# tsolomko/SWCompression

Hardware: AMD Instinct MI355X
Metric: decompressed GiB/s (higher is better)
Workload: dtype u8; 1 GPU; 100000 x 64 KiB gzip members (BASELINE configs[1]; 4096 distinct, tiled at distinct addresses); codec=deflate, units_per_gpu=100000, unit_bytes=65536, compressed_bytes_per_gpu=2122936095, decompressed_bytes_per_gpu=6553600000, parallelism=1 x independent shards (weak scaling)

## Files before the change

### swcompression_amd/csrc/inflate_sync.h

```cpp
#ifndef SWC_INFLATE_SYNC_H
#define SWC_INFLATE_SYNC_H

#include "inflate_lane.h"
#include "simt.h"
#include "sync_round.h"

namespace swc {
namespace inflate {

#ifndef SWC_SYNC_LIT_BITS
#define SWC_SYNC_LIT_BITS 10
#endif
constexpr int kSyncLitBits = SWC_SYNC_LIT_BITS, kSyncDistBits = 8;
constexpr uint32_t kSyncChunk = SWC_SYNC_CHUNK;
constexpr uint32_t kSyncRound = 64u * kSyncChunk;
constexpr uint32_t kSyncStage = (kSyncRound + 32u + 15u) & ~15u;
constexpr uint32_t kPosFail = 0xFFFFFFFFu;
#ifndef SWC_SYNC_WALK_BACK
#define SWC_SYNC_WALK_BACK 128
#endif
#ifndef SWC_COPY_REC
#define SWC_COPY_REC 16
#define SWC_COPY_LIT 8
#endif
constexpr uint32_t kSyncWalkBack = SWC_SYNC_WALK_BACK;
static_assert(kSyncChunk % 4 == 0 && kSyncChunk >= 36, "sub-chunks are whole dwords");

#ifndef SWC_SYNC_NO_PAIRS
#define SWC_SYNC_NO_PAIRS 0
#endif
constexpr uint32_t kEntLenBit = (uint32_t)kSyncLitBits + 2u;
constexpr uint32_t kEntNotLen = ((1u << (kSyncLitBits - kSyncDistBits)) - 1u) << (kSyncDistBits + 2), kEntLen = 1u << kEntLenBit, kEntLit = 1u << 13, kEntDist = 1u << 29, kEntStop = 1u << 30, kEntTog = 1u << 31;
static_assert(kSyncLitBits > kSyncDistBits && kEntLenBit <= 12u, "the entry keeps bits 10 .. 12 for the table switch");
constexpr uint32_t kEntBaseShift = 14, kEntPosMask = kEntTog | kEntStop | 31u;
constexpr uint32_t kLitMask4 = ((1u << kSyncLitBits) - 1u) << 2, kDistMask4 = ((1u << kSyncDistBits) - 1u) << 2;
static_assert(kEntLen == 4u << kSyncLitBits, "the length flag is the byte offset of the distance table");
static_assert((kLitMask4 & ~kEntNotLen) == kDistMask4, "the masks differ in the not-length bits");
constexpr uint32_t kInvLit = 2u | kEntNotLen | kEntStop, kInvDist = kInvLit | kEntTog;
constexpr uint32_t kEntShShift = 23, kEntPairBit = 28, kEntPair = SWC_SYNC_NO_PAIRS ? 0u : 1u << kEntPairBit, kEntPairLenShift = 16, kPairLenMax = 127;
SWC_HD uint32_t make_entry(uint32_t clen, uint32_t ext, uint32_t kind, uint32_t mant, uint32_t sh) {
    const uint32_t c = (clen + ext + 2u) | ((clen + 2u) << 5);
    const uint32_t v = SWC_SYNC_NO_PAIRS ? (mant << sh) << kEntBaseShift : (mant << kEntBaseShift) | (sh << kEntShShift);
    return kind == 1 ? c | kEntNotLen | kEntLit | v
         : kind == 2 ? c | kEntLen | kEntTog | v
         : kind == 3 ? c | kEntNotLen | kEntStop
                     : c | kEntNotLen | kEntDist | kEntTog | v;
}
SWC_HD uint32_t ent_bits(uint32_t e) { return (e & 31u) - 2u; }
SWC_HD uint32_t ent_code_bits(uint32_t e) { return ((e >> 5) & 31u) - 2u; }
SWC_HD bool ent_is_eob(uint32_t e) { return (e & kEntStop) != 0u && (e & 31u) > 2u; }
SWC_HD bool ent_is_link(uint32_t e) { return (e & kEntPosMask) == 0u; }
SWC_HD bool ent_is_pair(uint32_t e) { return (e & kEntPair) != 0u; }
SWC_HD uint32_t ent_pair_len(uint32_t e) { return bfe32(e, kEntPairLenShift, 7); }
SWC_HD uint32_t ent_base(uint32_t e) {
    if (SWC_SYNC_NO_PAIRS) return bfe32(e, kEntBaseShift, 15);
    return bfe32(e, kEntBaseShift, ent_is_pair(e) ? 2u : 9u) << bfe32(e, kEntShShift, 4);
}
SWC_HD uint32_t pair_entry(uint32_t e, uint32_t idx, const uint32_t* dlut) {
    if (SWC_SYNC_NO_PAIRS || ent_is_link(e) || (e & (kEntLen | kEntStop)) != kEntLen) return 0u;
    const uint32_t nl = ent_bits(e), cl = ent_code_bits(e);
    if (nl >= (uint32_t)kSyncLitBits) return 0u;
    const uint32_t r = (uint32_t)kSyncLitBits - nl;
    const uint32_t len = ent_base(e) + ((idx >> cl) & ((1u << (nl - cl)) - 1u));
    if (len > kPairLenMax) return 0u;
    const uint32_t de = dlut[(idx >> nl) & ((1u << kSyncDistBits) - 1u)];
    if (ent_is_link(de) || (de & (kEntDist | kEntStop)) != kEntDist) return 0u;
    const uint32_t d = ent_code_bits(de);
    if (d > r) return 0u;
    const uint32_t c2 = nl + d + 2u, n2 = c2 + (ent_bits(de) - d);
    return n2 | (c2 << 5) | kEntNotLen | kEntDist | kEntPair | (len << kEntPairLenShift) | (de & ((3u << kEntBaseShift) | (15u << kEntShShift)));
}

SWC_HD uint32_t entry_of_symbol(bool dist, uint32_t sym, uint32_t d) {
    if (!dist) {
        if (sym < 256) return make_entry(d, 0, 1, sym, 0);
        if (sym == 256) return make_entry(d, 0, 3, 0, 0);
        if (sym > 285) return kInvLit;
        const uint32_t s = sym - 257u;
        const uint32_t e = s < 8 || s == 28 ? 0u : (s >> 2) - 1u;
        const uint32_t base = s < 8 ? 3u + s : s == 28 ? 258u : 3u + ((4u + (s & 3u)) << e);
        return make_entry(d, e, 2, base, 0);
    }
    if (sym > 29) return kInvDist;
    const uint32_t e = sym < 4 ? 0u : (sym >> 1) - 1u;
    return make_entry(d, e, 0, sym < 4 ? sym : 2u + (sym & 1u), e);
}

constexpr int kAuxLim = 0, kAuxSlot = 16, kAuxStart = 32, kAuxCount = 48 , kAuxOver = 49, kAuxTable = 52;
constexpr int kAuxLit = 0, kAuxDist = kAuxTable, kAuxWords = 2 * kAuxTable;
constexpr uint32_t kSpillSyms = 512, kSpillSub = 1536, kSubLds = 184, kSubMax = (uint32_t)(lzr::kProvSpillBytes - kSpillSub) / 4u;
constexpr uint32_t kSymDist = 288;
static_assert(kAuxWords * 4 <= (int)kSpillSyms && kSpillSyms + 2 * (288 + 32) <= kSpillSub && kSubMax < 4096u, "spill layout");

struct SyncLds {
    alignas(16) uint8_t stage[kSyncStage];
    uint32_t lut[(1 << kSyncLitBits) + (1 << kSyncDistBits)];
    uint32_t sub[kSubLds];
};
#if SWC_SYNC_CHUNK == 68 && SWC_SYNC_LIT_BITS == 10
static_assert(sizeof(SyncLds) == 10240, "16 waves per CU: the wave's LDS must stay within 160 KB / 16");
#endif
constexpr uint32_t kHdrLens = 0;
constexpr uint32_t kHdrRun = 320;
constexpr uint32_t kHdrClLut = 512;
constexpr uint32_t kHdrSorted = 640;
constexpr uint32_t kHdrRank = 1280;
constexpr uint32_t kHdrIn = 1280;
constexpr uint32_t kHdrPt = 1280;
constexpr uint32_t kHdrTab = 3840;
static_assert(kHdrTab + 2 * 33 * 4 <= kSyncStage && kHdrPt + 2 * 1280 <= kHdrTab, "header scratch fits the stage");

enum { kSyncEob = 0, kSyncBail = 1, kSyncBailCap = 2 };
#if defined(SWC_HOST_EMULATION)
inline uint64_t g_sync_stats[8];
#define SWC_SYNC_STAT(i, n) (g_sync_stats[i] += (n))
inline uint64_t g_sync_iters = 0, g_sync_wave[4] = {0, 0, 0, 0}, g_sync_passmax = 0, g_sync_it0 = 0;
inline uint8_t g_sync_long[4096];
#define SWC_SYNC_ITER() (g_sync_iters++)
#define SWC_SYNC_LONG() (g_sync_long[(g_sync_iters - 1 - g_sync_it0) & 4095] = 1)
#define SWC_SYNC_LANE_BEGIN(first) if (first) { g_sync_passmax = 0; for (auto& h_ : g_sync_long) h_ = 0; } g_sync_it0 = g_sync_iters;
#define SWC_SYNC_LANE_END(last, k) { if (g_sync_iters - g_sync_it0 > g_sync_passmax) g_sync_passmax = g_sync_iters - g_sync_it0; if (last) { g_sync_wave[k] += g_sync_passmax; for (auto h_ : g_sync_long) g_sync_wave[3] += h_; } }
#else
#define SWC_SYNC_STAT(i, n) ((void)0)
#define SWC_SYNC_ITER() ((void)0)
#define SWC_SYNC_LONG() ((void)0)
#define SWC_SYNC_LANE_BEGIN(first)
#define SWC_SYNC_LANE_END(last, k)
#endif
enum { kFlagEob = 1u, kFlagFail = 2u, kFlagTrap = 4u, kFlagSlow = 8u };
#if defined(SWC_PROFILE) && defined(__HIP_DEVICE_COMPILE__)
struct SyncProf {
    uint64_t acc[16] = {0, 0, 0, 0, 0, 0, 0, 0, 0, 0, 0, 0, 0, 0, 0, 0};
    uint64_t tlast = 0;
};
#define SWC_SP(pp, k) { const uint64_t t_ = __builtin_readcyclecounter(); (pp).acc[k] += t_ - (pp).tlast; (pp).tlast = t_; }
#define SWC_SPC(pp, k, n) ((pp).acc[k] += (n))
#else
struct SyncProf {};
#define SWC_SP(pp, k)
#define SWC_SPC(pp, k, n)
#endif

struct SubTab {
    const SWC_AS_GLOBAL uint32_t* g;
};
struct Spill {
    SWC_AS_GLOBAL uint32_t* aux;
    SWC_AS_GLOBAL uint16_t* syms;
    SWC_AS_GLOBAL uint32_t* sub;
};

SWC_D uint32_t stage_bits(const SyncLds* sl, uint32_t p) {
    const uint32_t* w = (const uint32_t*)(sl->stage + ((p >> 3) & 0x1FFCu));
    return funnel32(w[1], w[0], p);
}
SWC_D uint32_t long_lookup(const SyncLds* sl, const SubTab st, uint32_t bits4, uint32_t link) {
    const uint32_t idx = bfe32(bits4, link >> 10, link >> 5);
    const uint32_t at = (link >> 18) + idx;
    return st.g ? st.g[at] : sl->sub[at < kSubLds ? at : 0u];
}
SWC_D uint32_t entry_at(const SyncLds* sl, const SubTab st, uint32_t pos, bool dist, uint32_t& bits4) {
    bits4 = stage_bits(sl, pos);
    uint32_t e = *(const uint32_t*)((const uint8_t*)sl->lut + ((bits4 & (dist ? kDistMask4 : kLitMask4)) | (dist ? kEntLen : 0u)));
    if (ent_is_link(e)) e = long_lookup(sl, st, bits4, e);
    return e;
}

template <bool LIT>
SWC_D int decode_sym_canon(BitReader& br, const Spill sp) {
    const SWC_AS_GLOBAL uint32_t* tb = sp.aux + (LIT ? kAuxLit : kAuxDist);
    const uint32_t c15 = brev32(br.peek32()) >> 17;
    uint32_t len = 16, idx = 0;
    if (tb[kAuxOver] == 0) {
        len = 1;
#pragma unroll 1
        for (int d = 1; d <= 15; d++) len += c15 >= tb[kAuxLim + d] ? 1u : 0u;
        if (len > 15) return -1;
        idx = (tb[kAuxSlot + len] + (c15 >> (15 - len))) & 0xFFFFu;
    } else {
#pragma unroll 1
        for (uint32_t d = 1; d <= 15; d++) {
            const uint32_t st = tb[kAuxStart + d], cnt = (tb[kAuxStart + d + 1] - st) & 0xFFFFu;
            const uint32_t fst = d == 1 ? 0u : tb[kAuxLim + d - 1] >> (15 - d);
            const uint32_t k0 = ((c15 >> (15 - d)) - fst) & ((1u << d) - 1u);
            if (k0 < cnt) {
                len = d;
                idx = st + k0 + (((cnt - 1u - k0) >> d) << d);
                break;
            }
        }
        if (len > 15) return -1;
    }
    if (len > br.bc) return -1;
    br.consume(len);
    if (idx >= (LIT ? 288u : 32u)) return -1;
    return (int)sp.syms[(LIT ? 0u : kSymDist) + idx];
}

SWC_D int careful_step(Lane& ln, const Spill sp) {
    BitReader& br = ln.br;
    br.refill();
    const int sym = decode_sym_canon<true>(br, sp);
    if (sym < 0) return SWC_E_DEFLATE_SYMBOL_NOT_FOUND;
    if (sym < 256) {
        ln.put_byte((uint8_t)sym);
        return SWC_OK;
    }
    if (sym == 256) return -1;
    if (sym > 285) return SWC_E_DEFLATE_WRONG_SYMBOL;
    const uint32_t s = (uint32_t)sym - 257u;
    uint32_t length;
    if (s < 8) {
        length = 3 + s;
    } else if (s == 28) {
        length = 258;
    } else {
        const uint32_t e = (s >> 2) - 1;
        if (br.bc < e) return SWC_E_DEFLATE_SYMBOL_NOT_FOUND;
        length = 3 + ((4 + (s & 3)) << e) + br.bits(e);
    }
    br.refill();
    const int dc = decode_sym_canon<false>(br, sp);
    if (dc < 0) return SWC_E_DEFLATE_SYMBOL_NOT_FOUND;
    if (dc > 29) return SWC_E_DEFLATE_WRONG_SYMBOL;
    uint32_t distance;
    if (dc < 4) {
        distance = 1 + (uint32_t)dc;
    } else {
        const uint32_t e = ((uint32_t)dc >> 1) - 1;
        if (br.bc < e) return SWC_E_DEFLATE_SYMBOL_NOT_FOUND;
        distance = 1 + ((2 + ((uint32_t)dc & 1)) << e) + br.bits(e);
    }
    if ((uint64_t)distance > ln.pos) {
        const uint32_t over = distance - (uint32_t)ln.pos;
        if (over > ln.back) return SWC_E_REF_TRAP;
        if (over > ln.reach) ln.reach = over;
    }
    ln.emit_match(length, distance);
    return SWC_OK;
}

SWC_D void table_from_counts(const uint32_t* cnt, SWC_AS_GLOBAL uint32_t* tb, uint32_t* first, uint32_t* start) {
    uint32_t v = 0, off = 0, over = 0;
    tb[kAuxLim] = 0; tb[kAuxSlot] = 0; tb[kAuxStart] = 0;
    first[0] = 0; start[0] = 0;
#pragma unroll 1
    for (int d = 1; d <= 15; d++) {
        const uint32_t c = cnt[d];
        tb[kAuxLim + d] = (v + c) << (15 - d);
        if (c != 0 && v + c > (1u << d)) over = 1;
        tb[kAuxSlot + d] = (off - v) & 0xFFFFu;
        tb[kAuxStart + d] = off;
        first[d] = v;
        start[d] = off;
        off += c;
        v = (v + c) << 1;
    }
    tb[kAuxCount] = off;
    tb[kAuxOver] = over;
    start[16] = off;
}

SWC_D bool sync_tables_from_lengths(SyncLds* sl, const Spill sp, int literals, int distances, SubTab& st, SyncProf& pf) {
    SWC_SP(pf, 0)
    using simt::PT;
    constexpr int N = kWave;
    const uint8_t* lens = sl->stage + kHdrLens;
    uint32_t* run = (uint32_t*)(sl->stage + kHdrRun);
    uint16_t* sorted = (uint16_t*)(sl->stage + kHdrSorted);
    uint16_t* rankb = (uint16_t*)(sl->stage + kHdrRank);
    uint16_t* pt = (uint16_t*)(sl->stage + kHdrPt);
    uint32_t* tab = (uint32_t*)(sl->stage + kHdrTab);
    const int total = literals + distances;
    st.g = nullptr;
    SIMT_BEGIN(t, N) if (t < 32) run[t] = 0; SIMT_END_WAVE
    PT<uint32_t, N> v, upd;
    PT<uint64_t, N> m;
    PT<bool, N> p;
#pragma unroll 1
    for (int g = 0; g * N < literals + N; g++) {
        const bool is_dist = g * N >= literals;
        const int s0 = is_dist ? literals : g * N, s_end = is_dist ? total : literals;
        SIMT_BEGIN(t, N) v[t] = s0 + t < s_end ? (uint32_t)lens[s0 + t] : 0u; m[t] = ~0ull; SIMT_END
#pragma unroll
        for (int k = 0; k < 4; k++) {
            SIMT_BEGIN(t, N) p[t] = ((v[t] >> k) & 1u) != 0u; SIMT_END
            const uint64_t b = simt::wave_ballot<N>(p);
            SIMT_BEGIN(t, N) m[t] &= p[t] ? b : ~b; SIMT_END
        }
        SIMT_BEGIN(t, N)
            upd[t] = 0;
            if (v[t] != 0u) {
                const uint32_t rank = (uint32_t)simt::popc64(m[t] & ((1ull << t) - 1ull)), cnt = (uint32_t)simt::popc64(m[t]);
                const uint32_t base = run[(is_dist ? 16u : 0u) + v[t]];
                rankb[s0 + t] = (uint16_t)(base + rank);
                if (rank == cnt - 1u) upd[t] = base + cnt;
            }
        SIMT_END_WAVE
        SIMT_BEGIN(t, N) if (upd[t] != 0u) run[(is_dist ? 16u : 0u) + v[t]] = upd[t]; SIMT_END_WAVE
    }
    SWC_SP(pf, 10)
    SIMT_BEGIN(t, N)
        if (t < 2) table_from_counts(run + 16 * t, sp.aux + (t ? kAuxDist : kAuxLit), tab + 33 * t, tab + 33 * t + 16);
    SIMT_END_WAVE
    SIMT_BEGIN(t, N)
        for (int s = t; s < total; s += N) {
            const uint32_t d = lens[s];
            if (d) {
                const bool dd = s >= literals;
                const uint32_t j = (dd ? kSymDist : 0u) + tab[(dd ? 33 : 0) + 16 + d] + rankb[s];
                const uint32_t sym = (uint32_t)(s - (dd ? literals : 0));
                if (j < kSymDist + 32u) { sorted[j] = (uint16_t)(sym | (d << 9)); sp.syms[j] = (uint16_t)sym; }
            }
        }
        for (int i = t; i < (1 << kSyncLitBits) + (1 << kSyncDistBits); i += N) sl->lut[i] = i < (1 << kSyncLitBits) ? kInvLit : kInvDist;
    SIMT_END_WAVE
    simt::vmem_fence();
    SWC_SP(pf, 11)
    if (sp.aux[kAuxLit + kAuxOver] != 0u || sp.aux[kAuxDist + kAuxOver] != 0u) return false;
    uint32_t used = 0, used_lit = 0;
    PT<uint32_t, N> sz, rv, ln2;
#pragma unroll 1
    for (int tbl = 0; tbl < 2; tbl++) {
        const uint32_t root = tbl ? (uint32_t)kSyncDistBits : (uint32_t)kSyncLitBits, rmask = (1u << root) - 1u;
        const uint32_t* first = tab + 33 * tbl;
        const uint32_t* start = first + 16;
        const uint32_t n_sym = start[16] < (tbl ? 32u : 288u) ? start[16] : (tbl ? 32u : 288u);
        const uint16_t* srt = sorted + (tbl ? kSymDist : 0u);
        uint32_t* lut = sl->lut + (tbl ? (1 << kSyncLitBits) : 0);
        uint16_t* ptt = pt + (tbl ? (1 << kSyncLitBits) : 0);
#pragma unroll 1
        for (uint32_t j0 = 0; j0 < n_sym; j0 += (uint32_t)N) {
            SIMT_BEGIN(t, N)
                const uint32_t j = j0 + (uint32_t)t;
                sz[t] = 0; ln2[t] = 0; rv[t] = 0;
                if (j < n_sym) {
                    const uint32_t w = srt[j], sym = w & 511u, d = w >> 9;
                    const uint32_t code = first[d] + (j - start[d]);
                    const uint32_t rev = brev32(code) >> (32u - d);
                    rv[t] = rev; ln2[t] = d;
                    if (d <= root) {
                        const uint32_t entry = entry_of_symbol(tbl != 0, sym, d);
                        for (uint32_t q = rev; q <= rmask; q += 1u << d) lut[q] = entry;
                    } else {
                        bool last = j + 1u == n_sym;
                        if (!last) {
                            const uint32_t w2 = srt[j + 1u], d2 = w2 >> 9;
                            const uint32_t rev2 = brev32(first[d2] + (j + 1u - start[d2])) >> (32u - d2);
                            last = (rev2 & rmask) != (rev & rmask);
                        }
                        if (last) sz[t] = 1u << (d - root);
                    }
                }
            SIMT_END
            PT<uint32_t, N> x = sz;
            simt::wave_scan_incl<N>(x);
            SIMT_BEGIN(t, N)
                if (sz[t] != 0u) {
                    const uint32_t at = used + x[t] - sz[t], k = ln2[t] - root, pre = rv[t] & rmask;
                    if (at + sz[t] <= kSubMax) {
                        ptt[pre] = (uint16_t)(at | (k << 12));
                        lut[pre] = (k << 5) | ((root + 2u) << 10) | (at << 18);
                    }
                }
            SIMT_END
            used += simt::wave_read<N>(x, N - 1);
        }
        if (tbl == 0) used_lit = used;
    }
    SWC_SP(pf, 12)
    if (used > kSubMax) return false;
    SWC_AS_GLOBAL uint32_t* subg = used > kSubLds ? sp.sub : nullptr;
    st.g = subg;
    simt::wave_fence();
#if !SWC_SYNC_NO_PAIRS
    SIMT_BEGIN(t, N)
        for (int i = t; i < (1 << kSyncLitBits); i += N) {
            const uint32_t pe2 = pair_entry(sl->lut[i], (uint32_t)i, sl->lut + (1 << kSyncLitBits));
            if (pe2 != 0u) sl->lut[i] = pe2;
        }
    SIMT_END
#endif
    SIMT_BEGIN(t, N)
        for (uint32_t i = (uint32_t)t; i < used; i += (uint32_t)N) {
            const uint32_t inv = i < used_lit ? kInvLit : kInvDist;
            if (subg) subg[i] = inv; else sl->sub[i] = inv;
        }
    SIMT_END_WAVE
    if (subg) simt::vmem_fence();
#pragma unroll 1
    for (int tbl = 0; tbl < 2; tbl++) {
        const uint32_t root = tbl ? (uint32_t)kSyncDistBits : (uint32_t)kSyncLitBits, rmask = (1u << root) - 1u;
        const uint32_t* first = tab + 33 * tbl;
        const uint32_t* start = first + 16;
        const uint32_t n_sym = start[16] < (tbl ? 32u : 288u) ? start[16] : (tbl ? 32u : 288u);
        if (start[root + 1] >= n_sym) continue;
        const uint16_t* srt = sorted + (tbl ? kSymDist : 0u);
        const uint16_t* ptt = pt + (tbl ? (1 << kSyncLitBits) : 0);
        SIMT_BEGIN(t, N)
            for (uint32_t j = start[root + 1] + (uint32_t)t; j < n_sym; j += (uint32_t)N) {
                const uint32_t w = srt[j], sym = w & 511u, d = w >> 9;
                const uint32_t rev = brev32(first[d] + (j - start[d])) >> (32u - d);
                const uint32_t entry = entry_of_symbol(tbl != 0, sym, d);
                const uint32_t pw = ptt[rev & rmask], at = pw & 0xFFFu, k = pw >> 12;
                for (uint32_t q = rev >> root; q < (1u << k); q += 1u << (d - root)) {
                    if (subg) subg[at + q] = entry; else sl->sub[at + q] = entry;
                }
            }
        SIMT_END
    }
    simt::wave_fence();
    if (subg) simt::vmem_fence();
    SWC_SP(pf, 13)
    return true;
}

SWC_D uint32_t walk_chunk(const SyncLds* sl, const SubTab st, uint32_t start, uint32_t chunk_end, uint32_t in_bits) {
    if (chunk_end > in_bits) chunk_end = in_bits;
    if (start >= in_bits) return kPosFail;
    uint32_t pos = start, tm = kLitMask4, tb = 0, e = 0;
    uint32_t c_notlen = kEntNotLen, c_dmask = kDistMask4;
    SWC_OPAQUE(c_notlen); SWC_OPAQUE(c_dmask);
    if (start < chunk_end) do {
        SWC_SYNC_STAT(4, 1);
        SWC_SYNC_ITER();
        const uint32_t bits4 = stage_bits(sl, pos);
        e = *(const uint32_t*)((const uint8_t*)sl->lut + and_or(bits4, tm, tb));
        uint32_t mm = e & kEntPosMask;
        if (mm == 0u) { SWC_SYNC_STAT(7, 1); SWC_SYNC_LONG(); e = long_lookup(sl, st, bits4, e); mm = e & kEntPosMask; }
        pos = pos + mm + 0xFFFFFFFEu;
        tm = and_or(e, c_notlen, c_dmask);
        tb = e & kEntLen;
    } while ((int32_t)pos < (int32_t)chunk_end);
    const uint32_t endb = pos & 0x3FFFFFFFu;
    const bool fail = ((pos & kEntStop) != 0u && !ent_is_eob(e)) || endb > in_bits;
    return fail ? kPosFail : endb;
}

struct ProvOut {
    uint32_t end, nlit, nrec, nout, flags, tail;
    int32_t need;
};
using sround::kProvRow;

template <bool NEED>
SWC_D void decode_chunk_prov(const SyncLds* sl, const SubTab st, uint32_t start, uint32_t chunk_end, uint32_t in_bits, gptr prov,
                             uint32_t lane, uint32_t run0, ProvOut& r) {
    const uint32_t rbase = 4u * lane, lbase = (uint32_t)lzr::kProvRecBytes + 4u * lane;
    uint32_t pos = start, tm = kLitMask4, tb = 0, e = 0;
    uint32_t plen = 0, run = run0, nl3 = 3, nout = 0, lb = 0;
    uint32_t roff = rbase + kProvRow;
    int32_t need = -0x40000000;
    uint32_t c_notlen = kEntNotLen, c_dmask = kDistMask4;
    int32_t c_m256 = -256;
    SWC_OPAQUE(c_notlen); SWC_OPAQUE(c_dmask); SWC_OPAQUE(c_m256);
#if !SWC_SYNC_NO_PAIRS
    int32_t c_m4 = -4;
    SWC_OPAQUE(c_m4);
#endif
    if (chunk_end > in_bits) chunk_end = in_bits;
    const bool dead = start >= in_bits;
    uint32_t w0 = 0, w1 = 0;
    if (!dead && start < chunk_end) { const uint32_t* w = (const uint32_t*)(sl->stage + ((pos >> 3) & 0x1FFCu)); w0 = w[0]; w1 = w[1]; }
    if (!dead && start < chunk_end) do {
        SWC_SYNC_STAT(5, 1);
        SWC_SYNC_ITER();
        const uint32_t bits4 = funnel32(w1, w0, pos);
        e = *(const uint32_t*)((const uint8_t*)sl->lut + and_or(bits4, tm, tb));
        uint32_t mm = e & kEntPosMask;
        if (mm == 0u) { SWC_SYNC_STAT(7, 1); SWC_SYNC_LONG(); e = long_lookup(sl, st, bits4, e); mm = e & kEntPosMask; }
        pos = pos + mm + 0xFFFFFFFEu;
        { const uint32_t* w = (const uint32_t*)(sl->stage + ((pos >> 3) & 0x1FFCu)); w0 = w[0]; w1 = w[1]; }
        tm = and_or(e, c_notlen, c_dmask);
        tb = e & kEntLen;
#if SWC_SYNC_NO_PAIRS
        const uint32_t val = (bfe32(bits4, 0, e) >> ((e >> 5) & 31u)) + bfe32(e, kEntBaseShift, 15);
        const uint32_t mlen = plen;
#else
        const uint32_t lp = bfe32(e, kEntPairLenShift, 7) & sbfe1(e, kEntPairBit);
        const uint32_t val = lshl_add_v(mad24(lp, c_m4, bfe32(e, kEntBaseShift, 9)), bfe32(e, kEntShShift, 4), bfe32(bits4, 0, e) >> ((e >> 5) & 31u));
        const uint32_t mlen = plen + lp;
#endif
        const uint32_t lit1 = bfe32(e, 13, 1);
        lb = alignbyte32(val, lb, lit1);
        nl3 += lit1;
        const uint32_t dm = sbfe1(e, 29);
        if (((nl3 & 3u) | (lit1 << 2)) == 7u) store_u32(prov + lshl_add<6>(nl3 & ~3u, lbase), lb);
        if (dm != 0u) store_u32(prov + roff, lshl_add<7>(mlen, lshl_add<16>(val, run)));
        roff = mad24(dm, c_m256, roff);
        if (NEED) {
            const int32_t nd = (int32_t)val - (int32_t)nout;
            need = (int32_t)bfi32(dm, (uint32_t)(nd > need ? nd : need), (uint32_t)need);
        }
        nout += lit1 + mlen;
        run = clear_if(dm, run + lit1);
        plen = val & sbfe1(e, kEntLenBit);
    } while ((int32_t)pos < (int32_t)chunk_end);
    const uint32_t nlit = nl3 - 3u;
    if (nlit & 3u) store_u32(prov + lshl_add<6>(nl3 & ~3u, lbase), lb);
    const uint32_t endb = pos & 0x3FFFFFFFu;
    uint32_t flags = 0;
    if (dead) flags = kFlagFail;
    else if (pos & kEntStop) flags = ent_is_eob(e) ? kFlagEob : kFlagFail;
    uint32_t tail = 0;
    if (run > 0) {
        if (flags & kFlagEob) tail = run;
        else { store_u32(prov + roff, lzr::make_lits(run)); roff += kProvRow; }
    }
    if (endb > in_bits) flags |= kFlagFail;
    if (nlit + run0 > lzr::kLitRunMax) flags |= kFlagSlow;
    r.end = (flags & kFlagFail) ? kPosFail : endb;
    r.nlit = nlit; r.nrec = (roff - rbase) / kProvRow - 1u; r.nout = nout; r.flags = flags; r.tail = tail; r.need = need;
}

SWC_D void copy_prov(gcptr plit, gcptr prec, uint32_t nlit, uint32_t nrec, gptr ldst, SWC_AS_GLOBAL uint32_t* rdst) {
    sround::copy_prov<SWC_COPY_REC, SWC_COPY_LIT, true>(plit, prec, nlit, nrec, ldst, rdst);
}

struct ChunkOut {
    uint32_t end;
    uint32_t nlit, nrec, nout;
    uint32_t flags;
    uint32_t over;
};
template <int MODE, bool BIG, bool CHK>
SWC_D void decode_chunk(const SyncLds* sl, const SubTab st, uint32_t start, uint32_t chunk_end, uint32_t in_bits, gptr lit_dst,
                        SWC_AS_GLOBAL uint32_t* rec_dst, uint64_t out_pos0, ChunkOut& r, uint32_t back = 0) {
    uint32_t pos = start;
    bool dist_next = false;
    uint32_t plen = 0, run = 0, nlit = 0, nrec = 0, nout = 0, flags = 0, over = 0;
    uint32_t lb = 0, lbn = 0;
    const uint32_t own = out_pos0 > 0x40000000ull ? 0x40000000u : (uint32_t)out_pos0;
    const uint32_t room = own + back;
    for (;;) {
        if (!dist_next && pos >= chunk_end) break;
        SWC_SYNC_STAT(4 + MODE, 1);
        SWC_SYNC_ITER();
        uint32_t bits4;
        const uint32_t e = entry_at(sl, st, pos, dist_next, bits4);
        const uint32_t n = ent_bits(e);
        if ((e & kEntStop) || (CHK && pos + n > in_bits)) {
            if (!ent_is_eob(e) || (CHK && pos + n > in_bits)) flags |= kFlagFail;
            else { pos += n; flags |= kFlagEob; }
            break;
        }
        const bool was_dist = dist_next || ent_is_pair(e);
        if (ent_is_pair(e)) plen = ent_pair_len(e);
        const uint32_t is_lit = (e >> 13) & 1u;
        const uint32_t val = (bfe32(bits4, 0, e) >> ((e >> 5) & 31u)) + ent_base(e) + (was_dist ? 1u : 0u);
        if (MODE != 0 && was_dist && val > own + nout) {
            if (val > room + nout) { flags |= kFlagTrap; break; }
            if (val - (own + nout) > over) over = val - (own + nout);
        }
        const bool big = BIG && was_dist && run > lzr::kLitRunMax;
        if (MODE == 1) {
            if (is_lit) {
                lb = funnel32(val, lb, 8);
                if (++lbn == 4) { store_u32(lit_dst, lb); lit_dst += 4; lbn = 0; }
            }
            if (was_dist) {
                if (big) *rec_dst++ = lzr::make_lits(run);
                *rec_dst++ = lzr::make_match(big ? 0u : run, plen, val);
            }
        }
        nlit += is_lit;
        nout += is_lit + (was_dist ? plen : 0u);
        nrec += was_dist ? (big ? 2u : 1u) : 0u;
        run = was_dist ? 0u : run + is_lit;
        plen = (e & kEntLen) ? val : plen;
        dist_next = (e & kEntLen) != 0u;
        pos += n;
    }
    if (run > 0) {
        nrec++;
        if (MODE == 1) *rec_dst++ = lzr::make_lits(run);
    }
    if (MODE == 1) {
        for (uint32_t i = 0; i < lbn; i++) lit_dst[i] = (uint8_t)(lb >> (8 * (4u - lbn + i)));
    }
    r.end = (flags & kFlagFail) ? kPosFail : pos;
    r.nlit = nlit; r.nrec = nrec; r.nout = nout;
    r.flags = flags;
    r.over = over;
}

template <int N>
SWC_D void stage_round(SyncLds* sl, gcptr in, uint32_t in_len, uint32_t B, uint32_t first_start, simt::PT<uint32_t, N>& start) {
    using simt::PT;
    constexpr uint32_t kParts = (kSyncStage + 16u * N - 1u) / (16u * N);
    PT<uint64_t, N> sa[kParts], sb[kParts];
    PT<uint32_t, N> sp[kParts];
    SIMT_BEGIN(t, N)
#pragma unroll
        for (uint32_t k = 0; k < kParts; k++) {
            const uint32_t o = 16u * (uint32_t)t + k * 16u * N;
            uint64_t a = 0, b = 0;
            uint32_t prev = 0;
            const uint64_t at = (uint64_t)B + o;
            if (o < kSyncStage) {
                if (at + 16 <= in_len) {
                    a = load_u64(in + at); b = load_u64(in + at + 8);
                    if (o != 0) prev = load_u32(in + at - 4);
                } else {
                    for (uint32_t q = 0; q < 8; q++) if (at + q < in_len) a |= (uint64_t)in[at + q] << (8 * q);
                    for (uint32_t q = 0; q < 8; q++) if (at + 8 + q < in_len) b |= (uint64_t)in[at + 8 + q] << (8 * q);
                    if (o != 0) for (uint32_t q = 0; q < 4; q++) if (at - 4 + q < in_len) prev |= (uint32_t)in[at - 4 + q] << (8 * q);
                }
            }
            sa[k][t] = a; sb[k][t] = b; sp[k][t] = prev;
        }
    SIMT_END
    SIMT_BEGIN(t, N)
#pragma unroll
        for (uint32_t k = 0; k < kParts; k++) {
            const uint32_t o = 16u * (uint32_t)t + k * 16u * N;
            if (o < kSyncStage) {
                uint32_t* st32 = (uint32_t*)(sl->stage + o);
                const uint64_t a = sa[k][t], b = sb[k][t];
                const uint32_t w0 = (uint32_t)a, w1 = (uint32_t)(a >> 32), w2 = (uint32_t)b, w3 = (uint32_t)(b >> 32);
                st32[0] = funnel32(w0, sp[k][t], 30); st32[1] = funnel32(w1, w0, 30); st32[2] = funnel32(w2, w1, 30); st32[3] = funnel32(w3, w2, 30);
            }
        }
        start[t] = t == 0 ? first_start : (uint32_t)t * kSyncChunk * 8u - kSyncWalkBack;
    SIMT_END_WAVE
}
SWC_D bool redo_lane(int t, uint32_t& start, uint32_t pe, bool have) {
    const bool todo = t == 0 ? !have : pe != kPosFail && (start != pe || !have);
    if (todo && t != 0) start = pe;
    return todo;
}
SWC_D bool stopped_in_front(uint32_t start, uint32_t chunk_end) { return start + kSyncChunk * 8u < chunk_end; }
template <class R>
SWC_D void nothing_taken(R& r) {
    r = R{};
    r.end = kPosFail; r.flags = kFlagFail;
}
template <int N>
SWC_D bool prov_turn(int t, const SyncLds* sl, const SubTab st, uint32_t in_bits, gptr prov, bool need, uint32_t run0,
                     simt::PT<uint32_t, N>& start, const simt::PT<uint32_t, N>& pe, simt::PT<bool, N>& have, simt::PT<uint32_t, N>& endp,
                     simt::PT<uint32_t, N>& c_lit, simt::PT<uint32_t, N>& c_rec, simt::PT<uint32_t, N>& c_out, simt::PT<uint32_t, N>& flg,
                     simt::PT<uint32_t, N>& c_tail, simt::PT<uint32_t, N>& c_need) {
    if (!redo_lane(t, start[t], pe[t], have[t])) return false;
    ProvOut r;
    const uint32_t ce = ((uint32_t)t + 1u) * kSyncChunk * 8u;
    if (stopped_in_front(start[t], ce)) nothing_taken(r);
    else if (need) decode_chunk_prov<true>(sl, st, start[t], ce, in_bits, prov, (uint32_t)t, run0, r);
    else decode_chunk_prov<false>(sl, st, start[t], ce, in_bits, prov, (uint32_t)t, run0, r);
    endp[t] = r.end; c_lit[t] = r.nlit; c_rec[t] = r.nrec; c_out[t] = r.nout; flg[t] = r.flags;
    c_tail[t] = r.tail; c_need[t] = (uint32_t)r.need;
    have[t] = true;
    return true;
}

#ifndef SWC_TEAM_WAVES
#define SWC_TEAM_WAVES 6
#endif
#if defined(SWC_HOST_EMULATION)
inline uint64_t g_team_adopted = 0;
#define SWC_TEAM_STAT() (g_team_adopted++)
#else
#define SWC_TEAM_STAT() ((void)0)
#endif
constexpr int kTeamWaves = SWC_TEAM_WAVES;
constexpr uint32_t kTeamStride = 63u * kSyncChunk;
constexpr size_t kTeamProvBytes = lzr::kProvRecBytes + lzr::kProvLitBytes;
struct TeamRound {
    uint32_t c_lit[kWave], c_rec[kWave];
    uint32_t nv, eob, ok;
    uint32_t start1;
    uint32_t end_last, tail_last;
    uint32_t tot_lit, tot_rec, tot_out;
    uint32_t mneed;
    uint32_t adopt, nrec_base;
    uint64_t nlit_base;
};
struct TeamShared {
    uint32_t cmd;
    uint32_t gen;
    uint32_t B, in_len;
    uint64_t in, subg;
    uint64_t lits, recs;
    uint32_t hgen[kTeamWaves];
    TeamRound r[kTeamWaves - 1];
};
struct Team {
    TeamShared* sh = nullptr;
    SyncLds* lds = nullptr;
    gptr scratch = nullptr;
    int helpers = 0;
    uint32_t gen = 0;
};

SWC_D void team_helper_round(const Team& tm, int h) {
    using simt::PT;
    constexpr int N = kWave;
    TeamShared* sh = tm.sh;
    SyncLds* sl = tm.lds + h;
    TeamRound& R = sh->r[h - 1];
    const uint32_t in_len = simt::uniform(sh->in_len);
    const uint64_t B64 = (uint64_t)simt::uniform(sh->B) + (uint64_t)h * kTeamStride;
    gcptr in = (gcptr)(uintptr_t)simt::uniform(sh->in);
    const SubTab st{(const SWC_AS_GLOBAL uint32_t*)(uintptr_t)simt::uniform(sh->subg)};
    gptr prov = tm.scratch + (size_t)(h - 1) * kTeamProvBytes;
    if (B64 + 2u * kSyncChunk >= (uint64_t)in_len) {
        SIMT_BEGIN(t, N) if (t == 0) { R.ok = 0; R.nv = 0; R.eob = 0; R.adopt = 0; } SIMT_END_WAVE
        return;
    }
    const uint32_t B = (uint32_t)B64;
    if (simt::uniform(sh->hgen[h]) != simt::uniform(sh->gen)) {
        const SyncLds* msl = tm.lds;
        constexpr int kLutWords = (int)(sizeof(sl->lut) / 4), kSubWords = (int)(sizeof(sl->sub) / 4);
        SIMT_BEGIN(t, N)
            for (int i = t; i < kLutWords; i += N) sl->lut[i] = msl->lut[i];
            for (int i = t; i < kSubWords; i += N) sl->sub[i] = msl->sub[i];
            if (t == 0) sh->hgen[h] = sh->gen;
        SIMT_END_WAVE
    }
    const uint64_t left = (uint64_t)(in_len - B) * 8;
    const uint32_t in_bits = left > 0x3FFFFFFFull ? 0x3FFFFFFFu : (uint32_t)left;
    PT<uint32_t, N> start, endp, pe, c_lit, c_rec, c_out, flg, c_tail, c_need, x_lit, x_rec, x_out, xs;
    PT<bool, N> pb, have;
    stage_round<N>(sl, in, in_len, B, 0u, start);
    SIMT_BEGIN(t, N)
        const uint32_t ce = ((uint32_t)t + 1u) * kSyncChunk * 8u;
        endp[t] = walk_chunk(sl, st, start[t], ce, in_bits);
        flg[t] = 0; have[t] = t == 0;
        c_lit[t] = c_rec[t] = c_out[t] = c_tail[t] = 0; c_need[t] = 0;
    SIMT_END
    uint32_t nv = 0;
    bool ok = true, eob = false;
    for (;;) {
        const sround::Chain ch = sround::chain_check<N>(pe, start, endp, have, flg, 0u, kFlagEob);
        nv = ch.nv;
        SIMT_BEGIN(t, N) pb[t] = (flg[t] & (kFlagFail | kFlagSlow)) != 0 || (t == 0 && endp[t] == kPosFail); SIMT_END
        if (simt::wave_ballot<N>(pb) & sround::lanes_below(nv)) { ok = false; break; }
        if (ch.E < 64) { eob = true; break; }
        if (ch.b == 64) break;
        SIMT_BEGIN(t, N)
            prov_turn<N>(t, sl, st, in_bits, prov, true, 0u, start, pe, have, endp, c_lit, c_rec, c_out, flg, c_tail, c_need);
        SIMT_END
    }
    const sround::Totals tot = sround::lane_offsets<N>(1u, nv, c_lit, c_rec, c_out, x_lit, x_rec, x_out);
    SIMT_BEGIN(t, N)
        const bool v = t >= 1 && (uint32_t)t < nv;
        const int32_t shortfall = (int32_t)c_need[t] - (int32_t)(x_out[t] - c_out[t]);
        xs[t] = v ? (uint32_t)shortfall + 0x80000000u : 0u;
    SIMT_END
    simt::wave_scan_max_incl<N>(xs);
    const uint32_t mneed = simt::wave_read<N>(xs, N - 1);
    const uint32_t last = nv >= 1u ? nv - 1u : 0u;
    const uint32_t end_last = simt::wave_read<N>(endp, (int)last), tail_last = simt::wave_read<N>(c_tail, (int)last), start1 = simt::wave_read<N>(start, 1);
    SIMT_BEGIN(t, N)
        const bool v = t >= 1 && (uint32_t)t < nv;
        R.c_lit[t] = v ? c_lit[t] : 0u; R.c_rec[t] = v ? c_rec[t] : 0u;
        if (t == 0) {
            R.nv = nv; R.eob = eob ? 1u : 0u; R.ok = ok && nv >= 2u ? 1u : 0u;
            R.adopt = 0u;
            R.start1 = start1; R.end_last = end_last; R.tail_last = tail_last;
            R.tot_lit = tot.lit; R.tot_rec = tot.rec; R.tot_out = tot.out; R.mneed = mneed;
        }
    SIMT_END_WAVE
}
SWC_D void team_helper_copy(const Team& tm, int h, gptr lits, SWC_AS_GLOBAL uint32_t* recs) {
    using simt::PT;
    constexpr int N = kWave;
    const TeamRound& R = tm.sh->r[h - 1];
    if (simt::uniform(R.adopt) == 0u) return;
    gptr hp = tm.scratch + (size_t)(h - 1) * kTeamProvBytes;
    const uint64_t nlit = ((uint64_t)simt::uniform((uint32_t)(R.nlit_base >> 32)) << 32) | simt::uniform((uint32_t)R.nlit_base);
    const uint32_t nrec = simt::uniform(R.nrec_base);
    PT<uint32_t, N> c_lit, c_rec, x_lit, x_rec;
    SIMT_BEGIN(t, N) c_lit[t] = R.c_lit[t]; c_rec[t] = R.c_rec[t]; x_lit[t] = c_lit[t]; x_rec[t] = c_rec[t]; SIMT_END
    simt::wave_scan_incl<N>(x_lit);
    simt::wave_scan_incl<N>(x_rec);
    SIMT_BEGIN(t, N)
        if (c_lit[t] | c_rec[t]) {
            copy_prov(hp + lzr::kProvRecBytes + 4u * (uint32_t)t, hp + 4u * (uint32_t)t, c_lit[t], c_rec[t],
                      lits + nlit + (x_lit[t] - c_lit[t]), recs + nrec + (x_rec[t] - c_rec[t]));
        }
    SIMT_END
}

SWC_D void team_begin(Team& tm, gcptr in, uint32_t in_len, uint32_t B, const SubTab st, gptr lits, SWC_AS_GLOBAL uint32_t* recs) {
    TeamShared* sh = tm.sh;
    SIMT_BEGIN(t, kWave)
        if (t == 0) { sh->cmd = 1u; sh->gen = tm.gen; sh->B = B; sh->in_len = in_len; sh->in = (uint64_t)(uintptr_t)in; sh->subg = (uint64_t)(uintptr_t)st.g; sh->lits = (uint64_t)(uintptr_t)lits; sh->recs = (uint64_t)(uintptr_t)recs; }
    SIMT_END_WAVE
#if defined(__HIP_DEVICE_COMPILE__)
    __syncthreads();
#endif
}
SWC_D void team_end(Team& tm) {
#if defined(__HIP_DEVICE_COMPILE__)
    __syncthreads();
#else
    for (int h = 1; h <= tm.helpers; h++) team_helper_round(tm, h);
#endif
}
SWC_D void team_go(Team& tm, gptr lits, SWC_AS_GLOBAL uint32_t* recs) {
#if defined(__HIP_DEVICE_COMPILE__)
    simt::wave_fence();
    __syncthreads();
// ... 545 lines not shown
```

Before: 459.8 GiB/s.

## Decode a follow-up literal per iteration in the provisional sync decoder

Each loop iteration of decode_chunk_prov now does a second literal-table lookup right after the main symbol. If that lookup gives a plain literal, it is consumed in the same iteration, so up to two symbols are decoded per trip through the serial loop. The literal packing, run tracking and output counting are reworked to handle two literals at once. This shortens the dependent chain per symbol, at the cost of an extra LDS lookup and more ALU work on every iteration, including those where the follow-up is not a literal. A variant that reuses the already-held stage words sits behind a macro.

```diff
diff --git a/swcompression_amd/csrc/inflate_sync.h b/swcompression_amd/csrc/inflate_sync.h
--- a/swcompression_amd/csrc/inflate_sync.h
+++ b/swcompression_amd/csrc/inflate_sync.h
@@ -29,12 +29,20 @@
 #ifndef SWC_SYNC_NO_PAIRS
 #define SWC_SYNC_NO_PAIRS 0
 #endif
+#ifndef SWC_SYNC_NO_FOLLOW
+#define SWC_SYNC_NO_FOLLOW 0
+#endif
+#ifndef SWC_SYNC_FOLLOW_HELD
+#define SWC_SYNC_FOLLOW_HELD 0
+#endif
+#define SWC_SYNC_FOLLOW (SWC_SYNC_NO_FOLLOW ? 0 : SWC_SYNC_FOLLOW_HELD ? 2 : 1)
 constexpr uint32_t kEntLenBit = (uint32_t)kSyncLitBits + 2u;
 constexpr uint32_t kEntNotLen = ((1u << (kSyncLitBits - kSyncDistBits)) - 1u) << (kSyncDistBits + 2), kEntLen = 1u << kEntLenBit, kEntLit = 1u << 13, kEntDist = 1u << 29, kEntStop = 1u << 30, kEntTog = 1u << 31;
 static_assert(kSyncLitBits > kSyncDistBits && kEntLenBit <= 12u, "the entry keeps bits 10 .. 12 for the table switch");
 constexpr uint32_t kEntBaseShift = 14, kEntPosMask = kEntTog | kEntStop | 31u;
 constexpr uint32_t kLitMask4 = ((1u << kSyncLitBits) - 1u) << 2, kDistMask4 = ((1u << kSyncDistBits) - 1u) << 2;
 static_assert(kEntLen == 4u << kSyncLitBits, "the length flag is the byte offset of the distance table");
+static_assert(((((uint32_t)kSyncLitBits + 2u) << 10) & kEntLen) != 0u && (kEntLit & (kEntLen | kEntNotLen)) == 0u, "a link has the literal bit AND the length bit, a literal only the first (the follow-up literal tells them apart by that)");
 static_assert((kLitMask4 & ~kEntNotLen) == kDistMask4, "the masks differ in the not-length bits");
 constexpr uint32_t kInvLit = 2u | kEntNotLen | kEntStop, kInvDist = kInvLit | kEntTog;
 constexpr uint32_t kEntShShift = 23, kEntPairBit = 28, kEntPair = SWC_SYNC_NO_PAIRS ? 0u : 1u << kEntPairBit, kEntPairLenShift = 16, kPairLenMax = 127;
@@ -446,9 +454,17 @@
 template <bool NEED>
 SWC_D void decode_chunk_prov(const SyncLds* sl, const SubTab st, uint32_t start, uint32_t chunk_end, uint32_t in_bits, gptr prov,
                              uint32_t lane, uint32_t run0, ProvOut& r) {
-    const uint32_t rbase = 4u * lane, lbase = (uint32_t)lzr::kProvRecBytes + 4u * lane;
+    const uint32_t rbase = 4u * lane;
+#if !SWC_SYNC_FOLLOW
+    const uint32_t lbase = (uint32_t)lzr::kProvRecBytes + 4u * lane;
+#endif
     uint32_t pos = start, tm = kLitMask4, tb = 0, e = 0;
+#if SWC_SYNC_FOLLOW
+    const uint32_t lbase4 = (uint32_t)lzr::kProvRecBytes - kProvRow + 4u * lane;
+    uint32_t plen = 0, run = run0, nl4 = 4, nout = 0, lb = 0;
+#else
     uint32_t plen = 0, run = run0, nl3 = 3, nout = 0, lb = 0;
+#endif
     uint32_t roff = rbase + kProvRow;
     int32_t need = -0x40000000;
     uint32_t c_notlen = kEntNotLen, c_dmask = kDistMask4;
@@ -469,10 +485,28 @@
         e = *(const uint32_t*)((const uint8_t*)sl->lut + and_or(bits4, tm, tb));
         uint32_t mm = e & kEntPosMask;
         if (mm == 0u) { SWC_SYNC_STAT(7, 1); SWC_SYNC_LONG(); e = long_lookup(sl, st, bits4, e); mm = e & kEntPosMask; }
+#if SWC_SYNC_FOLLOW == 2
+        const uint32_t wbase = pos & ~31u;
+#endif
         pos = pos + mm + 0xFFFFFFFEu;
+#if SWC_SYNC_FOLLOW == 2
+        const uint32_t fb4 = (uint32_t)((((uint64_t)w1 << 32) | w0) >> ((pos - wbase) & 63u));
+        const uint32_t fend = wbase + (65u - kEntLenBit) < chunk_end ? wbase + (65u - kEntLenBit) : chunk_end;
+#else
         { const uint32_t* w = (const uint32_t*)(sl->stage + ((pos >> 3) & 0x1FFCu)); w0 = w[0]; w1 = w[1]; }
+#endif
         tm = and_or(e, c_notlen, c_dmask);
         tb = e & kEntLen;
+#if SWC_SYNC_FOLLOW
+#if SWC_SYNC_FOLLOW != 2
+        const uint32_t fb4 = funnel32(w1, w0, pos);
+        const uint32_t fend = chunk_end;
+#endif
+        const uint32_t f = *(const uint32_t*)((const uint8_t*)sl->lut + (fb4 & kLitMask4));
+        const uint32_t fm = ((uint32_t)(pos < fend) & (uint32_t)((f & (kEntLit | kEntLen)) == kEntLit)) != 0u ? f : 2u;
+        pos = pos + (fm & 31u) + 0xFFFFFFFEu;
+        { const uint32_t* w = (const uint32_t*)(sl->stage + ((pos >> 3) & 0x1FFCu)); w0 = w[0]; w1 = w[1]; }
+#endif
 #if SWC_SYNC_NO_PAIRS
         const uint32_t val = (bfe32(bits4, 0, e) >> ((e >> 5) & 31u)) + bfe32(e, kEntBaseShift, 15);
         const uint32_t mlen = plen;
@@ -483,21 +517,38 @@
 #endif
         const uint32_t lit1 = bfe32(e, 13, 1);
         lb = alignbyte32(val, lb, lit1);
+        const uint32_t dm = sbfe1(e, 29);
+#if SWC_SYNC_FOLLOW
+        const uint32_t lit2 = bfe32(fm, 13, 1), byte2 = fm >> kEntBaseShift, nl4_0 = nl4, litn = lit1 + lit2;
+        nl4 += litn;
+        if ((nl4 ^ nl4_0) > 3u) store_u32(prov + lshl_add<6>(nl4 & ~3u, lbase4), alignbyte32(byte2, lb, clear_if(nl4, lit2)));
+        lb = alignbyte32(byte2, lb, lit2);
+#else
         nl3 += lit1;
-        const uint32_t dm = sbfe1(e, 29);
+        const uint32_t litn = lit1;
         if (((nl3 & 3u) | (lit1 << 2)) == 7u) store_u32(prov + lshl_add<6>(nl3 & ~3u, lbase), lb);
+#endif
         if (dm != 0u) store_u32(prov + roff, lshl_add<7>(mlen, lshl_add<16>(val, run)));
         roff = mad24(dm, c_m256, roff);
         if (NEED) {
             const int32_t nd = (int32_t)val - (int32_t)nout;
             need = (int32_t)bfi32(dm, (uint32_t)(nd > need ? nd : need), (uint32_t)need);
         }
-        nout += lit1 + mlen;
+        nout += litn + mlen;
+#if SWC_SYNC_FOLLOW
+        run = bfi32(dm, lit2, run + litn);
+#else
         run = clear_if(dm, run + lit1);
+#endif
         plen = val & sbfe1(e, kEntLenBit);
     } while ((int32_t)pos < (int32_t)chunk_end);
+#if SWC_SYNC_FOLLOW
+    const uint32_t nlit = nl4 - 4u;
+    if (nlit & 3u) store_u32(prov + lshl_add<6>((nl4 & ~3u) + 4u, lbase4), lb);
+#else
     const uint32_t nlit = nl3 - 3u;
     if (nlit & 3u) store_u32(prov + lshl_add<6>(nl3 & ~3u, lbase), lb);
+#endif
     const uint32_t endb = pos & 0x3FFFFFFFu;
     uint32_t flags = 0;
     if (dead) flags = kFlagFail;
```

After: 469.0 GiB/s, median of 6. +2.0%, better.
